# ssiu/flash-attention-turing

Measured on AMD Instinct MI355X. Metric: attention_fwd_tflops, higher is better.
Workload: dtype f16; 1 GPU; BASELINE configs[2] per GPU: fwd b=4 seq=16384 h=32 h_k=32 d=128 fp16 causal; global_batch=4, seq_len=16384, parallelism=batch-sharded x1, no collective

## Files before the change

flash-attention-turing_amd/csrc/fa_fwd_pp16.hip:

```cpp
#include "fa_device.hpp"
#include "fa_params.hpp"

#include <type_traits>

namespace fa {

constexpr int kFwdThreads = 512;
constexpr float kPpDeferLog2 = 6.0f;
#define FA_PP_MIN_WAVES(D, BN) 2
#ifndef FA_PP16_MFMA_ROWSUM
#define FA_PP16_MFMA_ROWSUM 1
#endif
#ifndef FA_PP16_ROLE_DMA
#define FA_PP16_ROLE_DMA 1
#endif
#ifndef FA_PP16_EXACT_TILES
#define FA_PP16_EXACT_TILES 16
#endif
#ifndef FA_PP16_EXACT_TILES_BF16
#define FA_PP16_EXACT_TILES_BF16 64
#endif
#ifndef FA_PP16_ABL
#define FA_PP16_ABL 0
#endif
#ifndef FA_PP16_DMA_DEBUG
#define FA_PP16_DMA_DEBUG 0
#endif
#ifndef FA_PP16_RACY
#define FA_PP16_RACY 0
#endif
#if FA_PP16_RACY && FA_PP16_ROLE_DMA
#error "FA_PP16_RACY is the symmetric-role form: build with -DFA_PP16_ROLE_DMA=0"
#endif
#ifndef FA_PP16_DMA_FUSED
#define FA_PP16_DMA_FUSED 1
#endif
#ifndef FA_PP16_SKIP_PAD
#define FA_PP16_SKIP_PAD 1
#endif
#ifndef FA_PP16_PF
#define FA_PP16_PF 2
#endif

#ifdef FA_FWD_TIMING
#define FA_FWD_STAMP(i) do { const uint64_t now_ = __builtin_amdgcn_s_memtime(); asm volatile("s_waitcnt lgkmcnt(0)" ::: "memory"); tacc[i] += (uint32_t)(now_ - tlast); tlast = now_; } while (0)
#else
#define FA_FWD_STAMP(i) do { } while (0)
#endif
template <typename T, int D, bool CAUSAL, int BN, int QB = 2>
__global__ __launch_bounds__(kFwdThreads, FA_PP_MIN_WAVES(D, BN)) void fa_fwd_pp16_kernel(const FwdKernelParams p) {
    constexpr int RW = 16 * QB, kFwdBlockM = 8 * RW;
    constexpr int KS = D / 32, DB = D / 16, ROWB = D * 2, SLOTS = D / 8;
    constexpr int kFwdBlockN = BN, NKB = BN / 16, NC = BN / 32;
    constexpr int TILEB = kFwdBlockN * ROWB;
    constexpr int RING = 3;
    constexpr int RINGB = 2 * RING * TILEB, STAGEB = kFwdBlockM * ROWB;
    constexpr bool ML = FA_PP16_MFMA_ROWSUM == 2 || (FA_PP16_MFMA_ROWSUM == 1 && std::is_same<T, _Float16>::value);
    __shared__ __attribute__((aligned(16))) char smem_raw[RINGB + STAGEB];
    FA_LDS char* smem = (FA_LDS char*)smem_raw;
    FA_LDS char* kring = smem;
    FA_LDS char* vring = smem + RING * TILEB;
    FA_LDS char* stage = smem + RINGB;

    const int tid = threadIdx.x, lane = tid & 63, g = lane >> 4, n16 = lane & 15;
    const int wave = __builtin_amdgcn_readfirstlane(tid >> 6);
    const int group = wave >> 2;
    const int pi_g = (0x2130 >> (4 * g)) & 3;
    const int pi2_g = (0x3120 >> (4 * g)) & 3;
    const int q_row_a = wave * RW + n16;
    const float c = p.scale_log2e;
    const uint32_t q_rowb = (uint32_t)(p.q.row * 2), k_rowb = (uint32_t)(p.k.row * 2),
                   v_rowb = (uint32_t)(p.v.row * 2), o_rowb = (uint32_t)(p.o.row * 2);

    int tile, batch, head, tiles_seq;
    if (!decode_work<kFwdBlockM>(blockIdx.x, p.n_q_tiles, p.varlen_slots, p.cu_seqlens_q, p.b, p.h, tile, batch, head, tiles_seq, p.group_heads)) return;
    if (CAUSAL) tile = tiles_seq - 1 - tile;

    int sq = p.seqlen_q, sk = p.seqlen_k;
    int64_t q_row0 = 0, k_row0 = 0;
    const bool varlen = p.cu_seqlens_q != nullptr;
    if (varlen) {
        const int q_beg = p.cu_seqlens_q[batch], k_beg = p.cu_seqlens_k[batch];
        sq = min(p.cu_seqlens_q[batch + 1] - q_beg, p.seqlen_q);
        sk = p.cu_seqlens_k[batch + 1] - k_beg;
        q_row0 = q_beg; k_row0 = k_beg;
    }
    if (tile * kFwdBlockM >= sq) return;
    const char* q_bh = (const char*)uniform_ptr((const T*)p.q_ptr + (varlen ? 0 : (int64_t)batch * p.q.batch) + q_row0 * p.q.row + (int64_t)head * p.q.head);
    char* o_bh = (char*)uniform_ptr((T*)p.o_ptr + (varlen ? 0 : (int64_t)batch * p.o.batch) + q_row0 * p.o.row + (int64_t)head * p.o.head);
    float* lse_bh = uniform_ptr(p.lse_ptr + ((int64_t)batch * p.h + head) * p.lse_row_stride);
    const int head_k = head / p.h_ratio;
    const srd_t k_srd = make_srd(uniform_ptr((const T*)p.k_ptr + (varlen ? 0 : (int64_t)batch * p.k.batch) + k_row0 * p.k.row + (int64_t)head_k * p.k.head),
                                 sk > 0 ? (uint32_t)(sk - 1) * k_rowb + ROWB : 0u);
    const srd_t v_srd = make_srd(uniform_ptr((const T*)p.v_ptr + (varlen ? 0 : (int64_t)batch * p.v.batch) + k_row0 * p.v.row + (int64_t)head_k * p.v.head),
                                 sk > 0 ? (uint32_t)(sk - 1) * v_rowb + ROWB : 0u);
    auto q_ptr_of = [&](int t) __attribute__((always_inline)) { return (const T*)(q_bh + (uint32_t)(t * kFwdBlockM) * q_rowb); };
    auto o_ptr_of = [&](int t) __attribute__((always_inline)) { return (T*)(o_bh + (uint32_t)(t * kFwdBlockM) * o_rowb); };
    auto rows_of = [&](int t) __attribute__((always_inline)) { return min(kFwdBlockM, sq - t * kFwdBlockM); };
    int m0 = 0, delta = 0, n_tiles = 0, n_main = 0;
    auto set_current = [&](int t) __attribute__((always_inline)) {
        m0 = t * kFwdBlockM;
        delta = sk - sq;
        n_tiles = (sk + kFwdBlockN - 1) / kFwdBlockN;
        if (CAUSAL) {
            const int max_key = m0 + rows_of(t) - 1 + delta;
            n_tiles = max_key < 0 ? 0 : min(n_tiles, max_key / kFwdBlockN + 1);
        }
        n_main = min(n_tiles, sk / kFwdBlockN);
        if (CAUSAL) n_main = min(n_main, max(0, (m0 + delta + 1) / kFwdBlockN));
    };

    constexpr int DPW = BN * SLOTS / 512;
    uint32_t dma_goff_k[DPW], dma_goff_v[DPW];
#pragma unroll
    for (int i = 0; i < DPW; ++i) {
        const int chunk = (wave * DPW + i) * 64 + lane;
        const int row = chunk / SLOTS, phys = chunk % SLOTS;
        const int slot = lds_tile_logical_slot<D>(row, phys);
        dma_goff_k[i] = row * k_rowb + slot * 16;
        dma_goff_v[i] = row * v_rowb + slot * 16;
    }
    const uint32_t dma_loff = (uint32_t)wave * DPW * 1024;
    const uint32_t lds_k0 = lds_addr(kring) + dma_loff, lds_v0 = lds_addr(vring) + dma_loff;
#if FA_PP16_ROLE_DMA
    constexpr int RPW = BN * SLOTS / 256;
    const uint32_t r_rowb = group ? v_rowb : k_rowb;
    uint32_t dma_goff_r[RPW];
#pragma unroll
    for (int i = 0; i < RPW; ++i) {
        const int chunk = ((wave & 3) * RPW + i) * 64 + lane, row = chunk / SLOTS, phys = chunk % SLOTS;
        dma_goff_r[i] = row * r_rowb + lds_tile_logical_slot<D>(row, phys) * 16;
    }
    const uint32_t lds_r0 = (group ? lds_addr(vring) : lds_addr(kring)) + (uint32_t)(wave & 3) * RPW * 1024;
#endif
    uint32_t k_rd[KS];
    {
        const int row = 4 * ((0x3120 >> (4 * (n16 >> 2))) & 3) + (n16 & 3);
#pragma unroll
        for (int ks = 0; ks < KS; ++ks) k_rd[ks] = lds_addr(kring) + lds_tile_off<D>(row, 4 * ks + pi_g);
    }
    uint32_t v_rd[DB];
#pragma unroll
    for (int db = 0; db < DB; ++db) v_rd[db] = lds_addr(vring) + lds_tile_off<D>(4 * pi2_g + (n16 >> 2), 2 * db + ((n16 & 3) >> 1)) + 8 * (n16 & 1);
#pragma unroll
    for (int ks = 0; ks < KS; ++ks) asm volatile("" : "+v"(k_rd[ks]));
#pragma unroll
    for (int db = 0; db < DB; ++db) asm volatile("" : "+v"(v_rd[db]));

    set_current(tile);
    if (n_tiles == 0) {
        const int rows_here = rows_of(tile);
        const rsrc_t o_rs = make_rsrc(uniform_ptr(o_ptr_of(tile)), (uint32_t)(rows_here - 1) * o_rowb + ROWB);
        constexpr int O_CHUNKS_DEAD = (RW * SLOTS) / 64;
#pragma unroll
        for (int i = 0; i < O_CHUNKS_DEAD; ++i) {
            const int chunk = lane + i * 64, row = wave * RW + chunk / SLOTS, slot = chunk % SLOTS;
            buf_store16(o_rs, (uint32_t)row * o_rowb + slot * 16, u32x4{0u, 0u, 0u, 0u});
        }
        if (lane < RW && wave * RW + lane < rows_here) lse_bh[tile * kFwdBlockM + wave * RW + lane] = 0.f;
        return;
    }

    u32x4 qf[KS][QB];
    {
        const rsrc_t q_rs = make_rsrc(uniform_ptr(q_ptr_of(tile)), (uint32_t)(rows_of(tile) - 1) * q_rowb + ROWB);
#pragma unroll
        for (int ks = 0; ks < KS; ++ks)
#pragma unroll
            for (int qb = 0; qb < QB; ++qb) qf[ks][qb] = buf_load16(q_rs, (uint32_t)(q_row_a + 16 * qb) * q_rowb + (4 * ks + pi_g) * 16);
    }

    f32x4 oacc[DB][QB];
#pragma unroll
    for (int db = 0; db < DB; ++db)
#pragma unroll
        for (int qb = 0; qb < QB; ++qb) oacc[db][qb] = f32x4{0.f, 0.f, 0.f, 0.f};
    float m_run[QB], l_run[QB];
    f32x4 lacc[QB];
#pragma unroll
    for (int qb = 0; qb < QB; ++qb) { m_run[qb] = kNegBig; l_run[qb] = 0.f; lacc[qb] = f32x4{0.f, 0.f, 0.f, 0.f}; }
    u32x4 ones_a = {LP<T>::kOnes2, LP<T>::kOnes2, LP<T>::kOnes2, LP<T>::kOnes2};
    if constexpr (ML) asm volatile("" : "+v"(ones_a));

    int ring_u = 0, ring_um1 = 2, ring_up1 = 1;
    auto dma_k_tile = [&](const srd_t& srd, int t, int slot) __attribute__((always_inline)) {
#pragma unroll
        for (int i = 0; i < (FA_PP16_DMA_FUSED && DPW == 2 ? 0 : DPW); ++i) dma16_to_lds_hidden<false>(srd, (uint32_t)(t * kFwdBlockN) * k_rowb + dma_goff_k[i], lds_k0 + slot * TILEB + i * 1024);
#if FA_PP16_DMA_FUSED
        if constexpr (DPW == 2) dma16x2_to_lds_hidden(srd, (uint32_t)(t * kFwdBlockN) * k_rowb, dma_goff_k[0], dma_goff_k[1], lds_k0 + slot * TILEB);
#endif
    };
    auto dma_v_tile = [&](const srd_t& srd, int t, int slot) __attribute__((always_inline)) {
#pragma unroll
        for (int i = 0; i < (FA_PP16_DMA_FUSED && DPW == 2 ? 0 : DPW); ++i) dma16_to_lds_hidden<false>(srd, (uint32_t)(t * kFwdBlockN) * v_rowb + dma_goff_v[i], lds_v0 + slot * TILEB + i * 1024);
#if FA_PP16_DMA_FUSED
        if constexpr (DPW == 2) dma16x2_to_lds_hidden(srd, (uint32_t)(t * kFwdBlockN) * v_rowb, dma_goff_v[0], dma_goff_v[1], lds_v0 + slot * TILEB);
#endif
    };

#if FA_PP16_ROLE_DMA
    const srd_t r_srd = group ? v_srd : k_srd;
    auto dma_role_tile = [&](int t, int slot) __attribute__((always_inline)) {
#pragma unroll
        for (int i = 0; i < (FA_PP16_DMA_FUSED && (RPW == 4 || RPW == 2) ? 0 : RPW); ++i) dma16_to_lds_hidden<false>(r_srd, (uint32_t)(t * kFwdBlockN) * r_rowb + dma_goff_r[i], lds_r0 + slot * TILEB + i * 1024);
#if FA_PP16_DMA_FUSED
        if constexpr (RPW == 4) dma16x4_to_lds_hidden(r_srd, (uint32_t)(t * kFwdBlockN) * r_rowb, dma_goff_r[0], dma_goff_r[1], dma_goff_r[2], dma_goff_r[3], lds_r0 + slot * TILEB);
        if constexpr (RPW == 2) dma16x2_to_lds_hidden(r_srd, (uint32_t)(t * kFwdBlockN) * r_rowb, dma_goff_r[0], dma_goff_r[1], lds_r0 + slot * TILEB);
#endif
    };
#endif

    if (n_tiles > 0) {
        dma_k_tile(k_srd, 0, 0);
        dma_v_tile(v_srd, 0, 0);
        dma_k_tile(k_srd, 1, 1);
    }
    asm volatile("s_waitcnt vmcnt(0)" ::: "memory");
    __syncthreads();
    if (group == 1) __syncthreads();

    f32x4 sacc[NKB][QB];
    u32x4 pf[NC][QB];
    const int wave_q_lo = m0 + wave * RW, wave_q_hi = wave_q_lo + RW - 1;

    constexpr int NPV = NC * DB, NQK = NKB * KS, NST = NPV + NQK, PF = FA_PP16_PF;
    auto m_frag = [&](int j, int slot_v, int slot_k) __attribute__((always_inline)) -> u32x4 {
#if FA_PP16_ABL & 8
        return qf[j % KS][(j >> 2) & 1];
#endif
        if (j < NPV) {
            const int db = j % DB, cch = j / DB;
            const u32x2 a0 = lds_read_tr8((const FA_LDS char*)(uintptr_t)v_rd[db], slot_v * TILEB + (32 * cch) * ROWB);
            const u32x2 a1 = lds_read_tr8((const FA_LDS char*)(uintptr_t)v_rd[db], slot_v * TILEB + (32 * cch + 16) * ROWB);
            return u32x4{a0.x, a0.y, a1.x, a1.y};
        }
        const int i = j - NPV, ks = i / NKB, kb = i % NKB;
        return lds_read16((const FA_LDS char*)(uintptr_t)k_rd[ks], slot_k * TILEB + 16 * kb * ROWB);
    };
    bool prev_ml = false;
    auto m_mfma = [&](auto jc, const u32x4& fr, auto lsc) __attribute__((always_inline)) {
        constexpr int j = decltype(jc)::value;
        if constexpr (j < NPV) {
            constexpr int db = j % DB, cch = j / DB;
#pragma unroll
            for (int qb = 0; qb < QB; ++qb) LP<T>::mfma16_acc(oacc[db][qb], fr, pf[cch][qb]);
            if constexpr (ML && db == DB - 1) {
                bool take;
                if constexpr (std::is_same<decltype(lsc), bool>::value) take = lsc;
                else take = decltype(lsc)::value;
                if (take) {
#pragma unroll
                    for (int qb = 0; qb < QB; ++qb) LP<T>::mfma16_acc(lacc[qb], ones_a, pf[cch][qb]);
                }
            }
        } else {
            constexpr int i = j - NPV, ks = i / NKB, kb = i % NKB;
            if constexpr (ks == 0) {
#pragma unroll
                for (int qb = 0; qb < QB; ++qb) LP<T>::mfma16_zero(sacc[kb][qb], fr, qf[ks][qb]);
            } else {
#pragma unroll
                for (int qb = 0; qb < QB; ++qb) LP<T>::mfma16_acc(sacc[kb][qb], fr, qf[ks][qb]);
            }
        }
    };
    u32x4 pre[PF];
    auto m_phase = [&](int slot_v, int slot_k, auto lsc) __attribute__((always_inline)) {
        u32x4 fr[NST];
        static_for<0, PF>([&](auto jc) { fr[decltype(jc)::value] = pre[decltype(jc)::value]; });
        static_for<0, NST>([&](auto jc) {
            constexpr int j = decltype(jc)::value;
            if constexpr (j + PF < NST) fr[j + PF] = m_frag(j + PF, slot_v, slot_k);
            __builtin_amdgcn_sched_barrier(0);
            m_mfma(jc, fr[j], lsc);
#if FA_PP16_ABL & 32
            if constexpr (!std::is_same<decltype(lsc), bool>::value) {
                if constexpr (decltype(lsc)::value && j < DB) {
                    constexpr int kb = NKB / 2 + j / 4, r0 = (j % 4) & 2, qb = j & 1;
                    const float e0 = fast_exp2(__builtin_fmaf(sacc[kb][qb][r0], c, -m_run[qb] * c));
                    const float e1 = fast_exp2(__builtin_fmaf(sacc[kb][qb][r0 + 1], c, -m_run[qb] * c));
                    const uint32_t w = LP<T>::pack2(e0, e1);
                    asm volatile("" ::"v"(w));
                }
            }
#endif
            __builtin_amdgcn_sched_barrier(0);
        });
    };
    auto m_prefetch = [&](int slot_v, int slot_k) __attribute__((always_inline)) {
#pragma unroll
        for (int j = 0; j < PF; ++j) pre[j] = m_frag(j, slot_v, slot_k);
    };
    auto pv_step = [&]() __attribute__((always_inline)) {
        static_for<0, NPV>([&](auto jc) { m_mfma(jc, m_frag(decltype(jc)::value, ring_um1, ring_u), prev_ml); });
    };
    auto qk_step = [&]() __attribute__((always_inline)) {
        static_for<NPV, NST>([&](auto jc) { m_mfma(jc, m_frag(decltype(jc)::value, ring_um1, ring_u), false); });
    };
    auto issue_dma_k = [&](int u) __attribute__((always_inline)) {
        if (u + 2 < n_tiles) dma_k_tile(k_srd, u + 2, ring_um1);
    };
    auto issue_dma_v = [&](int u) __attribute__((always_inline)) {
        if (u + 1 < n_tiles) dma_v_tile(v_srd, u + 1, ring_up1);
    };
    auto max4 = [&](float x) __attribute__((always_inline)) -> float {
        uint32_t u = __builtin_bit_cast(uint32_t, x);
        auto r = __builtin_amdgcn_permlane16_swap(u, u, false, false);
        x = fmaxf(__builtin_bit_cast(float, (uint32_t)r[0]), __builtin_bit_cast(float, (uint32_t)r[1]));
        return max_both_halves(x);
    };
    auto sum4 = [&](float x) __attribute__((always_inline)) -> float {
        uint32_t u = __builtin_bit_cast(uint32_t, x);
        auto r = __builtin_amdgcn_permlane16_swap(u, u, false, false);
        x = __builtin_bit_cast(float, (uint32_t)r[0]) + __builtin_bit_cast(float, (uint32_t)r[1]);
        return sum_both_halves(x);
    };
    auto softmax_step = [&](int u, auto masked, auto maybe_first, auto mlc, auto covered) __attribute__((always_inline)) {
        constexpr bool MLT = ML && decltype(mlc)::value;
        if constexpr (!decltype(covered)::value) asm volatile("s_nop 7\n\ts_nop 3" ::: "memory");
#pragma unroll
        for (int kb = 0; kb < NKB; ++kb)
#pragma unroll
            for (int qb = 0; qb < QB; ++qb) asm volatile("" : "+v"(sacc[kb][qb]));
        const int n0 = u * kFwdBlockN;
        if constexpr (decltype(masked)::value) {
            const bool need_mask = (n0 + kFwdBlockN > sk) || (CAUSAL && (n0 + kFwdBlockN - 1 > wave_q_lo + delta));
            if (need_mask) {
#pragma unroll
                for (int qb = 0; qb < QB; ++qb) {
                    const int lim = (CAUSAL ? min(sk - 1, m0 + q_row_a + 16 * qb + delta) : sk - 1) - n0 - 4 * pi2_g;
#pragma unroll
                    for (int kb = 0; kb < NKB; ++kb)
#pragma unroll
                        for (int r = 0; r < 4; ++r) sacc[kb][qb][r] = (16 * kb + r) <= lim ? sacc[kb][qb][r] : -INFINITY;
                }
            }
        }
        if constexpr (decltype(maybe_first)::value) {
            if (u == 0) {
#pragma unroll
                for (int qb = 0; qb < QB; ++qb) {
                    float mx = sacc[0][qb][0];
#pragma unroll
                    for (int kb = 0; kb < NKB; ++kb)
#pragma unroll
                        for (int r = 0; r < 4; ++r) mx = fmaxf(mx, sacc[kb][qb][r]);
                    m_run[qb] = fmaxf(kNegBig, max4(mx));
                }
            }
        }
        float ps[QB];
        auto pass = [&]() __attribute__((always_inline)) -> bool {
#pragma unroll
            for (int qb = 0; qb < QB; ++qb) {
                const float mc0 = m_run[qb] * c;
                ps[qb] = 0.f;
#pragma unroll
                for (int kb = 0; kb < NKB; ++kb) {
#if FA_PP16_ABL & 16
                    if (MLT && kb >= NKB / 2) continue;
#endif
#if FA_PP16_ABL & 4
                    const float p0 = sacc[kb][qb][0] * 0.01f + mc0 * 0.f, p1 = sacc[kb][qb][1] * 0.01f, p2 = sacc[kb][qb][2] * 0.01f, p3 = sacc[kb][qb][3] * 0.01f;
#else
                    const float p0 = fast_exp2(__builtin_fmaf(sacc[kb][qb][0], c, -mc0)), p1 = fast_exp2(__builtin_fmaf(sacc[kb][qb][1], c, -mc0));
                    const float p2 = fast_exp2(__builtin_fmaf(sacc[kb][qb][2], c, -mc0)), p3 = fast_exp2(__builtin_fmaf(sacc[kb][qb][3], c, -mc0));
#endif
                    if constexpr (!MLT) { ps[qb] += p0; ps[qb] += p1; ps[qb] += p2; ps[qb] += p3; }
                    if (kb & 1) { pf[kb >> 1][qb].z = LP<T>::pack2(p0, p1); pf[kb >> 1][qb].w = LP<T>::pack2(p2, p3); }
                    else { pf[kb >> 1][qb].x = LP<T>::pack2(p0, p1); pf[kb >> 1][qb].y = LP<T>::pack2(p2, p3); }
                }
            }
            if constexpr (MLT) {
                uint32_t t0, t1;
                if constexpr (QB != 2) {
                    uint32_t tq[QB];
#pragma unroll
                    for (int qb = 0; qb < QB; ++qb) {
                        tq[qb] = pk_max3_f16_bits(pf[0][qb].x, pf[0][qb].y, pf[0][qb].z);
#pragma unroll
                        for (int cch = 1; cch < NC; ++cch) {
                            tq[qb] = pk_max3_f16_bits(tq[qb], pf[cch - 1][qb].w, pf[cch][qb].x);
                            tq[qb] = pk_max3_f16_bits(tq[qb], pf[cch][qb].y, pf[cch][qb].z);
                        }
                    }
                    static_assert(QB == 2 || QB == 3, "guard merge written for three columns");
                    t0 = pk_max3_f16_bits(tq[0], tq[1], tq[QB - 1]);
                    t0 = pk_max3_f16_bits(t0, pf[NC - 1][0].w, pf[NC - 1][1].w);
                    t0 = pk_max3_f16_bits(t0, pf[NC - 1][QB - 1].w, pf[NC - 1][QB - 1].w);
                    (void)t1;
                } else if constexpr (NC == 2) {
                    t0 = pk_max3_f16_bits(pf[0][0].x, pf[0][0].y, pf[0][0].z); t1 = pk_max3_f16_bits(pf[0][1].x, pf[0][1].y, pf[0][1].z);
                    t0 = pk_max3_f16_bits(t0, pf[0][0].w, pf[1][0].x); t1 = pk_max3_f16_bits(t1, pf[0][1].w, pf[1][1].x);
                    t0 = pk_max3_f16_bits(t0, pf[1][0].y, pf[1][0].z); t1 = pk_max3_f16_bits(t1, pf[1][1].y, pf[1][1].z);
                    t0 = pk_max3_f16_bits(t0, pf[1][0].w, t1);
                    t0 = pk_max3_f16_bits(t0, pf[1][1].w, pf[1][1].w);
                } else {
                    t0 = pf[0][0].x; t1 = pf[0][1].x;
                    t0 = pk_max3_f16_bits(t0, pf[0][0].y, pf[0][0].z); t1 = pk_max3_f16_bits(t1, pf[0][1].y, pf[0][1].z);
#pragma unroll
                    for (int cch = 1; cch < NC; ++cch) {
                        t0 = pk_max3_f16_bits(t0, pf[cch - 1][0].w, pf[cch][0].x); t1 = pk_max3_f16_bits(t1, pf[cch - 1][1].w, pf[cch][1].x);
                        t0 = pk_max3_f16_bits(t0, pf[cch][0].y, pf[cch][0].z); t1 = pk_max3_f16_bits(t1, pf[cch][1].y, pf[cch][1].z);
                    }
                    t0 = pk_max3_f16_bits(t0, pf[NC - 1][0].w, pf[NC - 1][1].w);
                    t0 = pk_max3_f16_bits(t0, t1, t1);
                }
                const uint32_t both = max(t0, t0 << 16);
                return both > ((LP<T>::kBits64 << 16) | 0xffffu);
            } else {
                bool ok = true;
#pragma unroll
                for (int qb = 0; qb < QB; ++qb) ok = ok && ps[qb] <= 64.0f;
                return !ok;
            }
        };
        if constexpr (MLT) {
            if (__builtin_expect(__builtin_amdgcn_ballot_w64(pass()) != 0, 0)) {
                float mx[QB];
#pragma unroll
                for (int qb = 0; qb < QB; ++qb) {
                    mx[qb] = sacc[0][qb][0];
#pragma unroll
                    for (int kb = 0; kb < NKB; ++kb)
#pragma unroll
                        for (int r = 0; r < 4; ++r) mx[qb] = fmaxf(mx[qb], sacc[kb][qb][r]);
                    mx[qb] = max4(mx[qb]);
                }
                bool grew = false;
#pragma unroll
                for (int qb = 0; qb < QB; ++qb) grew = grew || (mx[qb] - m_run[qb]) * c > kPpDeferLog2;
                if (__builtin_amdgcn_ballot_w64(grew) != 0) {
#pragma unroll
                    for (int qb = 0; qb < QB; ++qb) {
                        const float m_new = fmaxf(m_run[qb], mx[qb]);
                        const float alpha = fast_exp2((m_run[qb] - m_new) * c);
                        m_run[qb] = m_new;
                        l_run[qb] *= alpha;
#pragma unroll
                        for (int r = 0; r < 4; ++r) lacc[qb][r] *= alpha;
#pragma unroll
                        for (int db = 0; db < DB; ++db)
#pragma unroll
                            for (int r = 0; r < 4; ++r) oacc[db][qb][r] *= alpha;
                    }
                    (void)pass();
                }
            }
            return;
        }
        for (int attempt = 0;; ++attempt) {
            const bool over = pass();
            if (attempt != 0 || __builtin_amdgcn_ballot_w64(over) == 0) break;
            float mx[QB];
#pragma unroll
            for (int qb = 0; qb < QB; ++qb) {
                mx[qb] = sacc[0][qb][0];
#pragma unroll
                for (int kb = 0; kb < NKB; ++kb)
#pragma unroll
                    for (int r = 0; r < 4; ++r) mx[qb] = fmaxf(mx[qb], sacc[kb][qb][r]);
                mx[qb] = max4(mx[qb]);
            }
            bool grew = false;
#pragma unroll
            for (int qb = 0; qb < QB; ++qb) grew = grew || (mx[qb] - m_run[qb]) * c > kPpDeferLog2;
            if (__builtin_amdgcn_ballot_w64(grew) == 0) break;
#pragma unroll
            for (int qb = 0; qb < QB; ++qb) {
                const float m_new = fmaxf(m_run[qb], mx[qb]);
                const float alpha = fast_exp2((m_run[qb] - m_new) * c);
                m_run[qb] = m_new;
                l_run[qb] *= alpha;
                if constexpr (ML) {
#pragma unroll
                    for (int r = 0; r < 4; ++r) lacc[qb][r] *= alpha;
                }
#pragma unroll
                for (int db = 0; db < DB; ++db)
#pragma unroll
                    for (int r = 0; r < 4; ++r) oacc[db][qb][r] *= alpha;
            }
        }
#pragma unroll
        for (int qb = 0; qb < QB; ++qb) l_run[qb] += ps[qb];
    };
    auto advance_ring = [&]() __attribute__((always_inline)) {
        ring_um1 = ring_u;
        ring_u = ring_up1;
        ring_up1 = ring_up1 == 2 ? 0 : ring_up1 + 1;
    };
    auto end_s_phase = [&]() __attribute__((always_inline)) {
        asm volatile("s_waitcnt vmcnt(0)" ::: "memory");
        __syncthreads();
    };
    auto epilogue = [&](int t) __attribute__((always_inline)) {
        asm volatile("s_nop 7\n\ts_nop 7" ::: "memory");
#pragma unroll
        for (int db = 0; db < DB; ++db)
#pragma unroll
            for (int qb = 0; qb < QB; ++qb) asm volatile("" : "+v"(oacc[db][qb]));
        const int rows_here = rows_of(t);
#pragma unroll
        for (int qb = 0; qb < QB; ++qb) {
            if constexpr (ML) asm volatile("" : "+v"(lacc[qb]));
            const float l_tot = ML ? sum4(l_run[qb]) + lacc[qb][0] : sum4(l_run[qb]);
            const float inv = l_tot != 0.f ? fast_rcp(l_tot) : 0.f;
            const float lse = l_tot != 0.f ? (m_run[qb] * c + fast_log2(l_tot)) * kLn2 : 0.f;
            const int row = q_row_a + 16 * qb;
            if (g == 0 && row < rows_here) lse_bh[t * kFwdBlockM + row] = lse;
#pragma unroll
            for (int db = 0; db < DB; ++db) {
                u32x2 w;
                w.x = LP<T>::pack2(oacc[db][qb][0] * inv, oacc[db][qb][1] * inv);
                w.y = LP<T>::pack2(oacc[db][qb][2] * inv, oacc[db][qb][3] * inv);
                lds_write8(stage, lds_tile_off<D>(row, 2 * db + (g >> 1)) + 8 * (g & 1), w);
            }
        }
        const rsrc_t o_rs = make_rsrc(uniform_ptr(o_ptr_of(t)), (uint32_t)(rows_here - 1) * o_rowb + ROWB);
        constexpr int O_CHUNKS = (RW * SLOTS) / 64;
#pragma unroll
        for (int i = 0; i < O_CHUNKS; ++i) {
            const int chunk = lane + i * 64, row = wave * RW + chunk / SLOTS, slot = chunk % SLOTS;
            buf_store16(o_rs, (uint32_t)row * o_rowb + slot * 16, lds_read16(stage, lds_tile_off<D>(row, slot)));
        }
    };
    using yes = std::integral_constant<bool, true>;
    using no = std::integral_constant<bool, false>;

    bool prev_active = false;
    auto iteration = [&](int u, auto masked) __attribute__((always_inline)) {
        bool active = true;
        if constexpr (decltype(masked)::value) active = !CAUSAL || (u * kFwdBlockN <= wave_q_hi + delta);
        if (prev_active) pv_step();
        if (active) qk_step();
        issue_dma_k(u);
        __syncthreads();
        issue_dma_v(u);
        if (active) softmax_step(u, masked, yes{}, no{}, no{});
        prev_active = active;
        prev_ml = false;
        end_s_phase();
        advance_ring();
    };

#ifdef FA_FWD_TIMING
    uint32_t tacc[6] = {0u, 0u, 0u, 0u, 0u, 0u}, tsteps = 0u;
    uint64_t tlast = 0;
#endif
    int u = 0;
    if (n_main > 0) {
        iteration(0, no{});
        if (n_main > 1) m_prefetch(ring_um1, ring_u);
        auto step_c = [&](int uu, auto um1, auto u0, auto up1, auto lsc, auto mlc) __attribute__((always_inline)) {
            constexpr int S_UM1 = decltype(um1)::value, S_U = decltype(u0)::value, S_UP1 = decltype(up1)::value;
            m_phase(S_UM1, S_U, lsc);
            FA_FWD_STAMP(0);
            __syncthreads();
            FA_FWD_STAMP(1);
#if FA_PP16_ROLE_DMA
#if FA_PP16_DMA_DEBUG == 1
            softmax_step(uu, no{}, no{}, mlc, no{});
            m_prefetch(S_U, S_UP1);
            dma_role_tile(uu + 1, S_UP1);
            asm volatile("s_waitcnt vmcnt(0)" ::: "memory");
            __syncthreads();
#else
#if FA_PP16_DMA_DEBUG == 2
            if (group == 1) asm volatile("s_sleep 64" ::: "memory");
#endif
#if !(FA_PP16_ABL & 2)
            dma_role_tile(uu + 2, S_UM1);
#endif
            FA_FWD_STAMP(2);
            softmax_step(uu, no{}, no{}, mlc, std::integral_constant<bool, FA_PP16_DMA_FUSED && !(FA_PP16_ABL & 2) && FA_PP16_SKIP_PAD && (BN * (D / 8) / 256 == 4 || BN * (D / 8) / 256 == 2)>{});
            FA_FWD_STAMP(3);
            m_prefetch(S_U, S_UP1);
#if !(FA_PP16_ABL & 3)
            asm volatile("s_waitcnt vmcnt(%0)" ::"n"(RPW) : "memory");
#endif
            FA_FWD_STAMP(4);
            __syncthreads();
            FA_FWD_STAMP(5);
#ifdef FA_FWD_TIMING
            ++tsteps;
#endif
#endif
#elif FA_PP16_RACY
#if FA_PP16_DMA_DEBUG == 1
            softmax_step(uu, no{}, no{}, mlc, no{});
            m_prefetch(S_U, S_UP1);
            dma_v_tile(v_srd, uu + 1, S_UP1);
            dma_k_tile(k_srd, uu + 1, S_UP1);
            asm volatile("s_waitcnt vmcnt(0)" ::: "memory");
            __syncthreads();
#else
            dma_v_tile(v_srd, uu + 1, S_UP1);
            dma_k_tile(k_srd, uu + 2, S_UM1);
            softmax_step(uu, no{}, no{}, mlc, no{});
            m_prefetch(S_U, S_UP1);
            asm volatile("s_waitcnt vmcnt(%0)" ::"n"(DPW) : "memory");
            __syncthreads();
#endif
#else
            if (uu + 2 < n_tiles) dma_k_tile(k_srd, uu + 2, S_UM1);
            if (uu + 1 < n_tiles) dma_v_tile(v_srd, uu + 1, S_UP1);
            softmax_step(uu, no{}, no{}, mlc, no{});
            m_prefetch(S_U, S_UP1);
            end_s_phase();
#endif
        };
        using i0 = std::integral_constant<int, 0>;
        using i1 = std::integral_constant<int, 1>;
        using i2 = std::integral_constant<int, 2>;
        u = 1;
#ifdef FA_FWD_TIMING
        tlast = __builtin_amdgcn_s_memtime();
        asm volatile("s_waitcnt lgkmcnt(0)" ::: "memory");
#endif
#if FA_PP16_ROLE_DMA
        const bool role_loop = n_main >= 4;
        if (role_loop && group == 1) dma_role_tile(2, 2);
#endif
        constexpr int kExactTiles = (std::is_same<T, _Float16>::value ? FA_PP16_EXACT_TILES : FA_PP16_EXACT_TILES_BF16) * 64 / BN;
        constexpr int kExact = ML ? 1 + 3 * ((kExactTiles + 1) / 3) : 0;
        if constexpr (ML) {
            for (; u + 3 <= n_main && u + 3 <= kExact; u += 3) {
                step_c(u, i0{}, i1{}, i2{}, no{}, no{});
                step_c(u + 1, i1{}, i2{}, i0{}, no{}, no{});
                step_c(u + 2, i2{}, i0{}, i1{}, no{}, no{});
            }
            if (u == kExact && u + 3 <= n_main) {
                step_c(u, i0{}, i1{}, i2{}, no{}, yes{});
                step_c(u + 1, i1{}, i2{}, i0{}, yes{}, yes{});
                step_c(u + 2, i2{}, i0{}, i1{}, yes{}, yes{});
                u += 3;
                for (; u + 3 <= n_main; u += 3) {
                    step_c(u, i0{}, i1{}, i2{}, yes{}, yes{});
                    step_c(u + 1, i1{}, i2{}, i0{}, yes{}, yes{});
                    step_c(u + 2, i2{}, i0{}, i1{}, yes{}, yes{});
                }
                prev_ml = true;
            }
        } else {
            for (; u + 3 <= n_main; u += 3) {
                step_c(u, i0{}, i1{}, i2{}, no{}, no{});
                step_c(u + 1, i1{}, i2{}, i0{}, no{}, no{});
                step_c(u + 2, i2{}, i0{}, i1{}, no{}, no{});
            }
        }
#if FA_PP16_ROLE_DMA
#if FA_PP16_DMA_DEBUG == 1
        if (role_loop && u > 1) dma_role_tile(u + 1, ring_up1);
#endif
        if (role_loop) asm volatile("s_waitcnt vmcnt(0)" ::: "memory");
#elif FA_PP16_RACY
#if FA_PP16_DMA_DEBUG == 1
        if (u > 1) dma_k_tile(k_srd, u + 1, ring_up1);
#endif
        asm volatile("s_waitcnt vmcnt(0)" ::: "memory");
#endif
        for (; u < n_main; ++u) {
            m_phase(ring_um1, ring_u, prev_ml);
            __syncthreads();
            issue_dma_k(u);
            issue_dma_v(u);
            softmax_step(u, no{}, no{}, no{}, no{});
            prev_ml = false;
            m_prefetch(ring_u, ring_up1);
            end_s_phase();
            advance_ring();
        }
    }
    for (; u < n_tiles; ++u) iteration(u, yes{});
    if (prev_active) pv_step();
    epilogue(tile);
#ifdef FA_FWD_TIMING
    asm volatile("s_waitcnt vmcnt(0)" ::: "memory");
    if (lane == 0) {
#pragma unroll
        for (int i = 0; i < 6; ++i) lse_bh[tile * kFwdBlockM + wave * RW + i] = (float)tacc[i];
        lse_bh[tile * kFwdBlockM + wave * RW + 6] = (float)tsteps;
        lse_bh[tile * kFwdBlockM + wave * RW + 7] = (float)tile;
    }
#endif
    if (group == 0) __syncthreads();
}

#ifndef FA_FWD_D128_QB
#define FA_FWD_D128_QB 2
#endif
#ifndef FA_FWD_D128_BN
#define FA_FWD_D128_BN 64
#endif
int fwd_pp16_block_m(int d) { return d == 128 ? 128 * FA_FWD_D128_QB : 256; }

hipError_t launch_fwd_pp16(const FwdKernelParams& kp, int dtype, uint32_t grid, hipStream_t stream) {
    if (grid == 0) return hipSuccess;
    if (kp.d == 64) {
        if (dtype == 0) {
            if (kp.is_causal) hipLaunchKernelGGL((fa_fwd_pp16_kernel<_Float16, 64, true, 128>), dim3(grid), dim3(kFwdThreads), 0, stream, kp);
            else hipLaunchKernelGGL((fa_fwd_pp16_kernel<_Float16, 64, false, 128>), dim3(grid), dim3(kFwdThreads), 0, stream, kp);
        } else {
            if (kp.is_causal) hipLaunchKernelGGL((fa_fwd_pp16_kernel<__bf16, 64, true, 128>), dim3(grid), dim3(kFwdThreads), 0, stream, kp);
            else hipLaunchKernelGGL((fa_fwd_pp16_kernel<__bf16, 64, false, 128>), dim3(grid), dim3(kFwdThreads), 0, stream, kp);
        }
        return hipGetLastError();
    }
    if (dtype == 0) {
        if (kp.is_causal) hipLaunchKernelGGL((fa_fwd_pp16_kernel<_Float16, 128, true, FA_FWD_D128_BN, FA_FWD_D128_QB>), dim3(grid), dim3(kFwdThreads), 0, stream, kp);
        else hipLaunchKernelGGL((fa_fwd_pp16_kernel<_Float16, 128, false, FA_FWD_D128_BN, FA_FWD_D128_QB>), dim3(grid), dim3(kFwdThreads), 0, stream, kp);
    } else {
        if (kp.is_causal) hipLaunchKernelGGL((fa_fwd_pp16_kernel<__bf16, 128, true, FA_FWD_D128_BN, FA_FWD_D128_QB>), dim3(grid), dim3(kFwdThreads), 0, stream, kp);
        else hipLaunchKernelGGL((fa_fwd_pp16_kernel<__bf16, 128, false, FA_FWD_D128_BN, FA_FWD_D128_QB>), dim3(grid), dim3(kFwdThreads), 0, stream, kp);
    }
    return hipGetLastError();
}

}
```

Before: 1282 TFLOP/s.

## Use role-split K/V DMA across all causal iterations with depth-two prefetch

For causal kernels, the masked-edge iterations and the generic tail loop now use the role-split DMA scheme: wave group 0 loads K tiles and group 1 loads V tiles into the ring. Each iteration requests tile u+2 and waits only on the older outstanding loads. The prologue now starts the first role DMA before loading Q, so the Q fetch overlaps the first tile transfer. Optional timing instrumentation for the edge phases is added behind FA_FWD_TIMING. The risks are ring-slot hazards under the new request/retire ordering and the extra vmcnt handling.

```diff
diff --git a/flash-attention-turing_amd/csrc/fa_fwd_pp16.hip b/flash-attention-turing_amd/csrc/fa_fwd_pp16.hip
--- a/flash-attention-turing_amd/csrc/fa_fwd_pp16.hip
+++ b/flash-attention-turing_amd/csrc/fa_fwd_pp16.hip
@@ -46,6 +46,15 @@
 #define FA_FWD_STAMP(i) do { const uint64_t now_ = __builtin_amdgcn_s_memtime(); asm volatile("s_waitcnt lgkmcnt(0)" ::: "memory"); tacc[i] += (uint32_t)(now_ - tlast); tlast = now_; } while (0)
 #else
 #define FA_FWD_STAMP(i) do { } while (0)
+#endif
+#ifdef FA_FWD_TIMING
+#define FA_FWD_EDGE_BEGIN() do { tedge_last = __builtin_amdgcn_s_memtime(); asm volatile("s_waitcnt lgkmcnt(0)" ::: "memory"); } while (0)
+#define FA_FWD_EDGE_STAMP(i) do { const uint64_t now_ = __builtin_amdgcn_s_memtime(); asm volatile("s_waitcnt lgkmcnt(0)" ::: "memory"); tedge[i] += (uint32_t)(now_ - tedge_last); tedge_last = now_; } while (0)
+#define FA_FWD_EDGE_COUNT(i) do { ++tedge_n[i]; } while (0)
+#else
+#define FA_FWD_EDGE_BEGIN() do { } while (0)
+#define FA_FWD_EDGE_STAMP(i) do { } while (0)
+#define FA_FWD_EDGE_COUNT(i) do { } while (0)
 #endif
 template <typename T, int D, bool CAUSAL, int BN, int QB = 2>
 __global__ __launch_bounds__(kFwdThreads, FA_PP_MIN_WAVES(D, BN)) void fa_fwd_pp16_kernel(const FwdKernelParams p) {
@@ -55,6 +64,7 @@
     constexpr int TILEB = kFwdBlockN * ROWB;
     constexpr int RING = 3;
     constexpr int RINGB = 2 * RING * TILEB, STAGEB = kFwdBlockM * ROWB;
+    constexpr bool EDGE_ROLE = FA_PP16_ROLE_DMA && CAUSAL;
     constexpr bool ML = FA_PP16_MFMA_ROWSUM == 2 || (FA_PP16_MFMA_ROWSUM == 1 && std::is_same<T, _Float16>::value);
     __shared__ __attribute__((aligned(16))) char smem_raw[RINGB + STAGEB];
     FA_LDS char* smem = (FA_LDS char*)smem_raw;
@@ -65,6 +75,11 @@
     const int tid = threadIdx.x, lane = tid & 63, g = lane >> 4, n16 = lane & 15;
     const int wave = __builtin_amdgcn_readfirstlane(tid >> 6);
     const int group = wave >> 2;
+#ifdef FA_FWD_TIMING
+    uint32_t tedge[5] = {0u, 0u, 0u, 0u, 0u}, tedge_n[2] = {0u, 0u};
+    uint64_t tedge_last;
+    FA_FWD_EDGE_BEGIN();
+#endif
     const int pi_g = (0x2130 >> (4 * g)) & 3;
     const int pi2_g = (0x3120 >> (4 * g)) & 3;
     const int q_row_a = wave * RW + n16;
@@ -161,28 +176,6 @@
         return;
     }
 
-    u32x4 qf[KS][QB];
-    {
-        const rsrc_t q_rs = make_rsrc(uniform_ptr(q_ptr_of(tile)), (uint32_t)(rows_of(tile) - 1) * q_rowb + ROWB);
-#pragma unroll
-        for (int ks = 0; ks < KS; ++ks)
-#pragma unroll
-            for (int qb = 0; qb < QB; ++qb) qf[ks][qb] = buf_load16(q_rs, (uint32_t)(q_row_a + 16 * qb) * q_rowb + (4 * ks + pi_g) * 16);
-    }
-
-    f32x4 oacc[DB][QB];
-#pragma unroll
-    for (int db = 0; db < DB; ++db)
-#pragma unroll
-        for (int qb = 0; qb < QB; ++qb) oacc[db][qb] = f32x4{0.f, 0.f, 0.f, 0.f};
-    float m_run[QB], l_run[QB];
-    f32x4 lacc[QB];
-#pragma unroll
-    for (int qb = 0; qb < QB; ++qb) { m_run[qb] = kNegBig; l_run[qb] = 0.f; lacc[qb] = f32x4{0.f, 0.f, 0.f, 0.f}; }
-    u32x4 ones_a = {LP<T>::kOnes2, LP<T>::kOnes2, LP<T>::kOnes2, LP<T>::kOnes2};
-    if constexpr (ML) asm volatile("" : "+v"(ones_a));
-
-    int ring_u = 0, ring_um1 = 2, ring_up1 = 1;
     auto dma_k_tile = [&](const srd_t& srd, int t, int slot) __attribute__((always_inline)) {
 #pragma unroll
         for (int i = 0; i < (FA_PP16_DMA_FUSED && DPW == 2 ? 0 : DPW); ++i) dma16_to_lds_hidden<false>(srd, (uint32_t)(t * kFwdBlockN) * k_rowb + dma_goff_k[i], lds_k0 + slot * TILEB + i * 1024);
@@ -210,14 +203,58 @@
     };
 #endif
 
-    if (n_tiles > 0) {
-        dma_k_tile(k_srd, 0, 0);
-        dma_v_tile(v_srd, 0, 0);
-        dma_k_tile(k_srd, 1, 1);
-    }
-    asm volatile("s_waitcnt vmcnt(0)" ::: "memory");
+#if FA_PP16_ROLE_DMA
+    if constexpr (EDGE_ROLE) dma_role_tile(0, 0);
+#endif
+
+    u32x4 qf[KS][QB];
+    {
+        const rsrc_t q_rs = make_rsrc(uniform_ptr(q_ptr_of(tile)), (uint32_t)(rows_of(tile) - 1) * q_rowb + ROWB);
+#pragma unroll
+        for (int ks = 0; ks < KS; ++ks)
+#pragma unroll
+            for (int qb = 0; qb < QB; ++qb) qf[ks][qb] = buf_load16(q_rs, (uint32_t)(q_row_a + 16 * qb) * q_rowb + (4 * ks + pi_g) * 16);
+    }
+
+    f32x4 oacc[DB][QB];
+#pragma unroll
+    for (int db = 0; db < DB; ++db)
+#pragma unroll
+        for (int qb = 0; qb < QB; ++qb) oacc[db][qb] = f32x4{0.f, 0.f, 0.f, 0.f};
+    float m_run[QB], l_run[QB];
+    f32x4 lacc[QB];
+#pragma unroll
+    for (int qb = 0; qb < QB; ++qb) { m_run[qb] = kNegBig; l_run[qb] = 0.f; lacc[qb] = f32x4{0.f, 0.f, 0.f, 0.f}; }
+    int ring_u = 0, ring_um1 = 2, ring_up1 = 1;
+    u32x4 ones_a = {LP<T>::kOnes2, LP<T>::kOnes2, LP<T>::kOnes2, LP<T>::kOnes2};
+    if constexpr (ML) asm volatile("" : "+v"(ones_a));
+
+    if constexpr (EDGE_ROLE) {
+        asm volatile("s_waitcnt vmcnt(0)" ::: "memory");
+#pragma unroll
+        for (int ks = 0; ks < KS; ++ks)
+#pragma unroll
+            for (int qb = 0; qb < QB; ++qb) asm volatile("" : "+v"(qf[ks][qb]));
+    } else {
+        if (n_tiles > 0) {
+            dma_k_tile(k_srd, 0, 0);
+            dma_v_tile(v_srd, 0, 0);
+            dma_k_tile(k_srd, 1, 1);
+        }
+        asm volatile("s_waitcnt vmcnt(0)" ::: "memory");
+    }
     __syncthreads();
+    FA_FWD_EDGE_STAMP(0);
+#if FA_PP16_ROLE_DMA && FA_PP16_DMA_DEBUG != 1
+    if constexpr (EDGE_ROLE) {
+#if FA_PP16_DMA_DEBUG == 2
+        if (group == 1) asm volatile("s_sleep 64" ::: "memory");
+#endif
+        if (1 < n_tiles) dma_role_tile(1, 1);
+    }
+#endif
     if (group == 1) __syncthreads();
+    FA_FWD_EDGE_BEGIN();
 
     f32x4 sacc[NKB][QB];
     u32x4 pf[NC][QB];
@@ -317,7 +354,14 @@
     };
     auto softmax_step = [&](int u, auto masked, auto maybe_first, auto mlc, auto covered) __attribute__((always_inline)) {
         constexpr bool MLT = ML && decltype(mlc)::value;
-        if constexpr (!decltype(covered)::value) asm volatile("s_nop 7\n\ts_nop 3" ::: "memory");
+        if constexpr (!decltype(covered)::value && !EDGE_ROLE) asm volatile("s_nop 7\n\ts_nop 3" ::: "memory");
+        if constexpr (!decltype(covered)::value && EDGE_ROLE) {
+#pragma unroll
+            for (int kb = 0; kb < NKB; ++kb)
+#pragma unroll
+                for (int qb = 0; qb < QB; ++qb) asm volatile("" : "+v"(sacc[kb][qb]));
+            asm volatile("s_nop 7\n\ts_nop 3" ::: "memory");
+        }
 #pragma unroll
         for (int kb = 0; kb < NKB; ++kb)
 #pragma unroll
@@ -494,6 +538,30 @@
         asm volatile("s_waitcnt vmcnt(0)" ::: "memory");
         __syncthreads();
     };
+#if FA_PP16_ROLE_DMA
+    auto edge_request = [&](int u) __attribute__((always_inline)) {
+#if FA_PP16_DMA_DEBUG != 1
+        if (u + 2 < n_tiles) {
+#if FA_PP16_DMA_DEBUG == 2
+            if (group == 1) asm volatile("s_sleep 64" ::: "memory");
+#endif
+            dma_role_tile(u + 2, ring_um1);
+        }
+#endif
+    };
+    auto edge_retire = [&](int u) __attribute__((always_inline)) {
+#if FA_PP16_DMA_DEBUG == 1
+        if (u == 0) {
+            if (1 < n_tiles) dma_role_tile(1, 1);
+        } else if (u + 1 < n_tiles) dma_role_tile(u + 1, ring_up1);
+        asm volatile("s_waitcnt vmcnt(0)" ::: "memory");
+#else
+        if (u + 2 < n_tiles) asm volatile("s_waitcnt vmcnt(%0)" ::"n"(RPW) : "memory");
+        else asm volatile("s_waitcnt vmcnt(0)" ::: "memory");
+#endif
+        __syncthreads();
+    };
+#endif
     auto epilogue = [&](int t) __attribute__((always_inline)) {
         asm volatile("s_nop 7\n\ts_nop 7" ::: "memory");
 #pragma unroll
@@ -534,13 +602,25 @@
         if constexpr (decltype(masked)::value) active = !CAUSAL || (u * kFwdBlockN <= wave_q_hi + delta);
         if (prev_active) pv_step();
         if (active) qk_step();
-        issue_dma_k(u);
-        __syncthreads();
-        issue_dma_v(u);
-        if (active) softmax_step(u, masked, yes{}, no{}, no{});
-        prev_active = active;
-        prev_ml = false;
-        end_s_phase();
+#if FA_PP16_ROLE_DMA
+        if constexpr (EDGE_ROLE) {
+            __syncthreads();
+            edge_request(u);
+            if (active) softmax_step(u, masked, yes{}, no{}, no{});
+            prev_active = active;
+            prev_ml = false;
+            edge_retire(u);
+        } else
+#endif
+        {
+            issue_dma_k(u);
+            __syncthreads();
+            issue_dma_v(u);
+            if (active) softmax_step(u, masked, yes{}, no{}, no{});
+            prev_active = active;
+            prev_ml = false;
+            end_s_phase();
+        }
         advance_ring();
     };
 
@@ -551,6 +631,7 @@
     int u = 0;
     if (n_main > 0) {
         iteration(0, no{});
+        FA_FWD_EDGE_STAMP(1);
         if (n_main > 1) m_prefetch(ring_um1, ring_u);
         auto step_c = [&](int uu, auto um1, auto u0, auto up1, auto lsc, auto mlc) __attribute__((always_inline)) {
             constexpr int S_UM1 = decltype(um1)::value, S_U = decltype(u0)::value, S_UP1 = decltype(up1)::value;
@@ -620,7 +701,9 @@
 #endif
 #if FA_PP16_ROLE_DMA
         const bool role_loop = n_main >= 4;
-        if (role_loop && group == 1) dma_role_tile(2, 2);
+        if constexpr (!EDGE_ROLE) {
+            if (role_loop && group == 1) dma_role_tile(2, 2);
+        }
 #endif
         constexpr int kExactTiles = (std::is_same<T, _Float16>::value ? FA_PP16_EXACT_TILES : FA_PP16_EXACT_TILES_BF16) * 64 / BN;
         constexpr int kExact = ML ? 1 + 3 * ((kExactTiles + 1) / 3) : 0;
@@ -650,34 +733,63 @@
             }
         }
 #if FA_PP16_ROLE_DMA
+        if constexpr (!EDGE_ROLE) {
 #if FA_PP16_DMA_DEBUG == 1
-        if (role_loop && u > 1) dma_role_tile(u + 1, ring_up1);
-#endif
-        if (role_loop) asm volatile("s_waitcnt vmcnt(0)" ::: "memory");
+            if (role_loop && u > 1) dma_role_tile(u + 1, ring_up1);
+#endif
+            if (role_loop) asm volatile("s_waitcnt vmcnt(0)" ::: "memory");
+        }
+        (void)role_loop;
 #elif FA_PP16_RACY
 #if FA_PP16_DMA_DEBUG == 1
         if (u > 1) dma_k_tile(k_srd, u + 1, ring_up1);
 #endif
         asm volatile("s_waitcnt vmcnt(0)" ::: "memory");
 #endif
+        FA_FWD_EDGE_BEGIN();
         for (; u < n_main; ++u) {
             m_phase(ring_um1, ring_u, prev_ml);
             __syncthreads();
-            issue_dma_k(u);
-            issue_dma_v(u);
-            softmax_step(u, no{}, no{}, no{}, no{});
-            prev_ml = false;
-            m_prefetch(ring_u, ring_up1);
-            end_s_phase();
+#if FA_PP16_ROLE_DMA
+            if constexpr (EDGE_ROLE) {
+                edge_request(u);
+                softmax_step(u, no{}, no{}, no{}, no{});
+                prev_ml = false;
+                m_prefetch(ring_u, ring_up1);
+                edge_retire(u);
+            } else
+#endif
+            {
+                issue_dma_k(u);
+                issue_dma_v(u);
+                softmax_step(u, no{}, no{}, no{}, no{});
+                prev_ml = false;
+                m_prefetch(ring_u, ring_up1);
+                end_s_phase();
+            }
             advance_ring();
-        }
-    }
-    for (; u < n_tiles; ++u) iteration(u, yes{});
+            FA_FWD_EDGE_STAMP(3);
+            FA_FWD_EDGE_COUNT(1);
+        }
+    }
+    FA_FWD_EDGE_BEGIN();
+    for (; u < n_tiles; ++u) {
+        iteration(u, yes{});
+        FA_FWD_EDGE_STAMP(2);
+        FA_FWD_EDGE_COUNT(0);
+    }
     if (prev_active) pv_step();
+    if constexpr (EDGE_ROLE) asm volatile("s_waitcnt vmcnt(0)" ::: "memory");
     epilogue(tile);
 #ifdef FA_FWD_TIMING
     asm volatile("s_waitcnt vmcnt(0)" ::: "memory");
+    FA_FWD_EDGE_STAMP(4);
     if (lane == 0) {
+#pragma unroll
+        for (int i = 0; i < 5; ++i) lse_bh[tile * kFwdBlockM + wave * RW + 8 + i] = (float)tedge[i];
+        lse_bh[tile * kFwdBlockM + wave * RW + 13] = (float)tedge_n[0];
+        lse_bh[tile * kFwdBlockM + wave * RW + 14] = (float)tedge_n[1];
+        lse_bh[tile * kFwdBlockM + wave * RW + 15] = (float)n_tiles;
 #pragma unroll
         for (int i = 0; i < 6; ++i) lse_bh[tile * kFwdBlockM + wave * RW + i] = (float)tacc[i];
         lse_bh[tile * kFwdBlockM + wave * RW + 6] = (float)tsteps;
```

New measurement: 1294 TFLOP/s (median of 6 runs). Within noise of the previous version (+0.9%).
